# stardist/stardist

Measured on AMD Instinct MI355X. Metric: predict_instances() Mpix/s (2D) + Mvox/s (3D) end-to-end at 1/2/4/8 GPU, higher is better.
Workload: dtype f32

## Files before the change

stardist_amd/csrc/common.h:

```cpp
#pragma once
#include <hip/hip_runtime.h>
#include <stdint.h>
#include <stdio.h>
#include <string.h>

namespace sd {

char* err_buf();
void set_error(const char* fmt, ...);

#define SD_CHECK(expr)                                                                   \
  do {                                                                                   \
    hipError_t _e = (expr);                                                              \
    if (_e != hipSuccess) {                                                              \
      sd::set_error("%s:%d: %s -> %s", __FILE__, __LINE__, #expr, hipGetErrorString(_e)); \
      return -1;                                                                         \
    }                                                                                    \
  } while (0)

#define SD_LAUNCH_CHECK() SD_CHECK(hipGetLastError())

class Arena {
 public:
  int begin(hipStream_t stream);
  void* take(size_t bytes);
  template <typename T> T* take_n(size_t n) { return (T*)take((n ? n : 1) * sizeof(T)); }
  void release();
  size_t capacity() const;
 private:
  enum { kMaxChunks = 64 };
  void* base_[kMaxChunks] = {};
  size_t cap_[kMaxChunks] = {};
  int n_ = 0, cur_ = 0;
  size_t off_ = 0;
};
Arena& arena();

hipStream_t side_stream();

enum { kMaxDevices = 64 };
int resident_grid(const void* kernel, int threads, int* cache);

int cu_count();
int allow_dynamic_lds(const void* const* kernels, int n, int bytes, bool* done);

static inline int div_up(long long a, long long b) { return (int)((a + b - 1) / b); }

enum Option { OPT_NMS3D_VOLUME_BOUNDS, OPT_NMS3D_CONE_MAP, OPT_NMS3D_REFINE_MESH, OPT_PROBE_TIER, OPT_PROBE_NO_GENERAL, OPT_TRACE, OPT_NMS3D_TAIL_BATCH, OPT_NMS3D_SPLIT_EXACT, OPT_CONV_F16_WGS, OPT_NMS2D_PAIR_LANES, OPT_NMS2D_AREA_BOUNDS, OPT_NMS2D_DEFER_UNDECIDED, OPT_NMS2D_STRICT, OPT_NMS2D_NBR_SINGLE, OPT_NMS3D_NBR_SINGLE, OPT_NMS2D_DEFER_MAX, OPT_NMS3D_BOUNDS_REUSE, OPT_NMS3D_DEFER_EXACT, OPT_NMS3D_BOUNDS_LEAN, OPT_COUNT };
int option(Option o);

#ifdef SD_DEBUG_SWITCHES
int tuning_env(const char* name, int dflt);
#else
static inline int tuning_env(const char*, int dflt) { return dflt; }
#endif

}
```

stardist_amd/csrc/lib.hip:

```cpp
#include "common.h"
#include "../../include/stardist_hip.h"
#include <stdarg.h>
#include <stdlib.h>
#include <mutex>

namespace sd {

static thread_local char g_err[1024] = "";
char* err_buf() { return g_err; }
void set_error(const char* fmt, ...) {
  va_list ap;
  va_start(ap, fmt);
  vsnprintf(g_err, sizeof(g_err), fmt, ap);
  va_end(ap);
}

static int g_opt[OPT_COUNT] = {1, 1, 2, 1, 0, 0, 1, 3, 2, 64, 1, 2, 0, 1, 1, 16384, 1, 3, 1};
static const char* const g_opt_name[OPT_COUNT] = {"nms3d_volume_bounds", "nms3d_cone_map", "nms3d_refine_mesh", "probe_tier", "probe_no_general", "trace", "nms3d_tail_batch", "nms3d_split_exact", "conv_f16_workgroups_per_cu", "nms2d_pair_lanes", "nms2d_area_bounds", "nms2d_defer_undecided", "nms2d_strict", "nms2d_neighbours_single_pass", "nms3d_neighbours_single_pass", "nms2d_defer_max", "nms3d_bounds_reuse", "nms3d_defer_exact", "nms3d_bounds_lean"};
int option(Option o) { return g_opt[o]; }
#ifdef SD_DEBUG_SWITCHES
int tuning_env(const char* name, int dflt) { const char* e = getenv(name); return e ? atoi(e) : dflt; }
#endif

static Arena g_arena[kMaxDevices];
Arena& arena() {
  int d = 0;
  if (hipGetDevice(&d) != hipSuccess || d < 0 || d >= kMaxDevices) d = 0;
  return g_arena[d];
}

hipStream_t side_stream() {
  static std::mutex mu;
  static hipStream_t st[kMaxDevices] = {};
  int d = 0;
  if (hipGetDevice(&d) != hipSuccess || d < 0 || d >= kMaxDevices) { set_error("side_stream: no current device"); return nullptr; }
  std::lock_guard<std::mutex> lock(mu);
  if (!st[d] && hipStreamCreateWithFlags(&st[d], hipStreamNonBlocking) != hipSuccess) { st[d] = nullptr; set_error("side_stream: cannot create a stream"); }
  return st[d];
}

int resident_grid(const void* kernel, int threads, int* cache) {
  static std::mutex mu;
  int d = 0;
  if (hipGetDevice(&d) != hipSuccess || d < 0 || d >= kMaxDevices) { set_error("resident_grid: no current device"); return 0; }
  std::lock_guard<std::mutex> lock(mu);
  if (!cache[d]) {
    int per_cu = 0, cus = 0;
    if (hipOccupancyMaxActiveBlocksPerMultiprocessor(&per_cu, kernel, threads, 0) != hipSuccess ||
        hipDeviceGetAttribute(&cus, hipDeviceAttributeMultiprocessorCount, d) != hipSuccess || per_cu <= 0 || cus <= 0) {
      set_error("resident_grid: occupancy query failed");
      return 0;
    }
    cache[d] = per_cu * cus;
  }
  return cache[d];
}

int cu_count() {
  static std::mutex mu;
  static int n_cu[kMaxDevices] = {};
  int d = 0;
// ... 82 lines not shown
```

stardist_amd/csrc/nms2d.hip:

```cpp
#include <type_traits>

#include "common.h"
#include "clip_sweep.h"
#include "clip_beam.h"
#include "area_bounds.h"
#include "poly_pass.h"
#include "nms_rounds.h"
#include "../../include/stardist_hip.h"
#include <hipcub/hipcub.hpp>
#include <math.h>
#include <stdlib.h>
#include <vector>

namespace {

using sdclip::i64;

__device__ __forceinline__ float wave_min(float v) { for (int o = 32; o; o >>= 1) v = fminf(v, __shfl_xor(v, o)); return v; }
__device__ __forceinline__ float wave_max(float v) { for (int o = 32; o; o >>= 1) v = fmaxf(v, __shfl_xor(v, o)); return v; }
__device__ __forceinline__ i64 wave_sum(i64 v) { for (int o = 32; o; o >>= 1) v += __shfl_xor(v, o); return v; }

__global__ void __launch_bounds__(256) k_build(const float* __restrict__ dist, const float* __restrict__ pts,
                                               const float2* __restrict__ sincos, int N, int R,
                                               int* __restrict__ vx, int* __restrict__ vy, int4* __restrict__ bbox,
// ... 654 lines not shown
                                                             const unsigned char* __restrict__ decided, const unsigned char* __restrict__ state) {
  const unsigned long long n = *nPtr, first = firstPtr ? *firstPtr : 0u;
  for (unsigned long long t = first + (unsigned long long)blockIdx.x * 256 + threadIdx.x; t < n; t += (unsigned long long)gridDim.x * 256) {
    if (decided && decided[t]) continue;
    const int2 ij = pairs[t];
    if (pair_j_suppressed(state, ij)) continue;
    const unsigned int k = atomicAdd(&cursor[pair_bucket(pts, ij, key)], 1u);
    if (k < cap) order[k] = (unsigned int)t;
  }
}

__global__ void k_count_after(unsigned int* out, const unsigned int* total, const unsigned int* first) { *out = *total > *first ? *total - *first : 0u; }

}

namespace sd {
int clip_full_pairs(const int2* d_pairs, const unsigned int* d_idx, const unsigned int* d_n, unsigned int cap, int R, const int* d_vx, const int* d_vy,
                    const float* d_area, float thr, unsigned char* d_state, unsigned char* d_supp, unsigned int* d_errCount, hipStream_t stream);
}

namespace {
struct Counters { int nU, nK, nS, left; unsigned long long nPairs; unsigned int nSpill, nExact, nErr, nDecided, nSkipped; };

template <int MAXV, int SPREP>
struct BeamPath {
  typedef sdclip::PolyPrep<MAXV> Prep;
  static constexpr size_t prep_stride = sizeof(Prep);
  static constexpr bool two_tiers = MAXV == 32;
  static int prepare(const int* vx, const int* vy, int N, int R, sdarea::PolyProps* props, void* prep, hipStream_t s) {
    if constexpr (MAXV == 32) {
      if (sdpass::launch_poly_pass(vx, vy, N, R, props, prep, s)) { sd::set_error("sd_nms2d: launch of the per-polygon pass failed"); return -1; }
      return 0;
    } else {
      const size_t lds = sdclip::PrepWork<sdclip::LdsStorage<SPREP>, MAXV>::lds_bytes() + 64;
      hipLaunchKernelGGL((k_prepare<MAXV, SPREP>), dim3(sd::div_up(N, SPREP)), dim3(SPREP), lds, s, vx, vy, N, R, (Prep*)prep);
      SD_LAUNCH_CHECK();
      return 0;
    }
  }
  static int tier1(const int2* pairs, const unsigned int* idx, const unsigned long long* nPairs, const unsigned int* first, const void* prep, const float* area,
                   float thr, unsigned char* state, unsigned char* supp, PairQueues q, hipStream_t s) {
    const int lanes = sd::option(sd::OPT_NMS2D_PAIR_LANES);
    if (lanes == 32) {
      static const size_t lds32 = beam_lds_bytes<MAXV, 8, 6, 4, 32>();
      hipLaunchKernelGGL((k_pairs_beam<MAXV, 8, 6, 4, 32, unsigned long long>), dim3(256 * 8), dim3(32), lds32, s, pairs, idx, nPairs, first, (const Prep*)prep, area, thr, state, supp, q);
    } else if (lanes == 6464) {
// ... 87 lines not shown
  hipStream_t s = (hipStream_t)stream_;
  if (n_polys <= 0) return 0;
  if (n_rays < 1 || n_rays > 256) { sd::set_error("sd_nms2d_build: n_rays=%d unsupported (1..256)", n_rays); return -1; }
  sd::Arena& A = sd::arena();
  if (A.begin(s)) return -1;
  int* gstats = nullptr;
  if (launch_build(A, s, d_dist, d_points, n_polys, n_rays, d_vx, d_vy, (int4*)d_bbox, d_radius, d_area, &gstats, nullptr)) return -1;
  SD_CHECK(hipMemcpyAsync(d_gstats, gstats, 5 * sizeof(int), hipMemcpyDeviceToDevice, s));
  SD_CHECK(hipStreamSynchronize(s));
  return 0;
}

namespace {
struct SideEvents {
  hipEvent_t props = nullptr, prep = nullptr;
  ~SideEvents() { if (props) (void)hipEventDestroy(props); if (prep) (void)hipEventDestroy(prep); }
  int init() { SD_CHECK(hipEventCreateWithFlags(&props, hipEventDisableTiming)); SD_CHECK(hipEventCreateWithFlags(&prep, hipEventDisableTiming)); return 0; }
};

struct Nms2d {
  hipStream_t s; const float *dist, *pts; int N, R, use_kdtree, use_bbox; float thr; bool wantStats; sd::Arena& A;
  bool areaBounds = false, singlePass = false, ordered = false, decide = false, deferOn = false, trace = false;
  int tailT = -1, deferFrom = 0, keyMode = 2; unsigned int deferMax = 0;
  hipStream_t side = nullptr; sd::SideJoin sideJoin; SideEvents sideEv;
  Timer broadTimer, pairTimer, fullTimer, replayTimer;
  double ns_pairs = 0, ns_full = 0, ns_pre = 0; long long n_pair_launches = 0;
  int *vx = nullptr, *vy = nullptr, *candCell = nullptr, *gstats = nullptr; int4* bbox = nullptr; float *radius = nullptr, *area = nullptr;
  unsigned char* state = nullptr; void* prep = nullptr; size_t prepStride = 0; sdarea::PolyProps* props = nullptr;
  GridP g; NmsFlags f; float max_dist = 0, reach = 0;
  int by_bbox = 0, *cellStart = nullptr, *nbrCount = nullptr, *nbrLow = nullptr, *Ucur = nullptr; i64* nbrStart = nullptr; CellRec* cellRec = nullptr;
  void* scanTmp = nullptr; size_t scanBytes = 0; Deferred dfr{nullptr, nullptr, nullptr, nullptr, nullptr, 0};
  NbrLists L{}; i64 totalNbr = 0;
  unsigned long long pairCap = 0, *nOrdered = nullptr; int2* pairs = nullptr; unsigned char *decided = nullptr, *defKind = nullptr;
  unsigned int qCap = 0, *spillPairs = nullptr, *exactPairs = nullptr, *pairOrder = nullptr, *bucketHist = nullptr, *firstNew = nullptr, *nNewExact = nullptr, *nJoinDef = nullptr;
  int *Unext = nullptr, *K = nullptr, *Sl = nullptr, decideGrid = 0; Counters *d_cnt = nullptr, h;
  int nU = 0, rounds = 0; bool forceTail = false;
  i64 nDeferred = 0, nUndecDeferredUpper = 0, totalPairs = 0, totalExact = 0, totalSpill = 0, totalUndecDeferred = 0, totalDecided = 0, totalSkipped = 0;
  unsigned char* supp = nullptr; unsigned int* segStart = nullptr; int* segCnt = nullptr;

  Nms2d(hipStream_t s_, const float* dist_, const float* pts_, int N_, int R_, int use_kdtree_, int use_bbox_, float thr_, bool wantStats_)
      : s(s_), dist(dist_), pts(pts_), N(N_), R(R_), use_kdtree(use_kdtree_), use_bbox(use_bbox_), thr(thr_), wantStats(wantStats_), A(sd::arena()) {}

  int plan() {
    if (R < 1 || R > 256) { sd::set_error("sd_nms2d: n_rays=%d unsupported (1..256)", R); return -1; }
    if (A.begin(s)) return -1;
    if (wantStats && (broadTimer.init() || pairTimer.init() || fullTimer.init())) return -1;
    trace = wantStats && sd::option(sd::OPT_TRACE) != 0;
    areaBounds = R <= 32 && R >= 3 && sd::option(sd::OPT_NMS2D_AREA_BOUNDS) != 0 && sd::option(sd::OPT_NMS2D_STRICT) == 0;
    singlePass = sd::option(sd::OPT_NMS2D_NBR_SINGLE) != 0;
    static const bool pairSort = sd::tuning_env("SD_NMS_PAIR_SORT", 1) != 0;
    static const int pairKey = sd::tuning_env("SD_NMS_PAIR_KEY", 2);
    ordered = pairSort && R <= 32;
    keyMode = pairKey;
    decide = areaBounds && ordered;
    static const int tailDiv = sd::tuning_env("SD_NMS_TAIL_DIV", 6);
    static const int tailMax = sd::tuning_env("SD_NMS_TAIL_MAX", 65536);
    tailT = tailDiv > 0 ? ((N / tailDiv) < tailMax ? (N / tailDiv) : tailMax) : -1;
    static const bool deferEnv = sd::tuning_env("SD_NMS_DEFER", 1) != 0;
    deferOn = tailT >= 0 && deferEnv;
    deferFrom = (deferOn && decide) ? sd::option(sd::OPT_NMS2D_DEFER_UNDECIDED) : 0;
    deferMax = (unsigned int)(sd::option(sd::OPT_NMS2D_DEFER_MAX) > 0 ? sd::option(sd::OPT_NMS2D_DEFER_MAX) : 0);
    side = sd::side_stream();
    if (!side || sideEv.init()) return -1;
    return 0;
  }

  int build() {
    vx = A.take_n<int>((size_t)N * R);
    vy = A.take_n<int>((size_t)N * R);
    bbox = A.take_n<int4>(N);
    radius = A.take_n<float>(N);
    area = A.take_n<float>(N);
    state = A.take_n<unsigned char>(N);
    candCell = A.take_n<int>(N);
    prepStride = prep_stride(R);
    prep = A.take((size_t)N * prepStride);
    if (areaBounds) props = (sdarea::PolyProps*)A.take((size_t)N * sizeof(sdarea::PolyProps));
    if (!vx || !vy || !bbox || !radius || !area || !state || !candCell || !prep || (areaBounds && !props)) return -1;
    return launch_build(A, s, dist, pts, N, R, vx, vy, bbox, radius, area, &gstats, broadTimer.a);
  }

  int fork_side() {
    if (sideJoin.begin(s, side) || prepare_polys(vx, vy, N, R, props, prep, side)) return -1;
    SD_CHECK(hipEventRecord(sideEv.props, side));
    SD_CHECK(hipEventRecord(sideEv.prep, side));
    return 0;
  }

  int build_grid() {
    int gs[8];
    SD_CHECK(hipMemcpyAsync(gs, gstats, sizeof(gs), hipMemcpyDeviceToHost, s));
    SD_CHECK(hipStreamSynchronize(s));
    memcpy(&max_dist, &gs[0], 4);
    reach = (max_dist + 1.f) * 1.0001f + 1e-3f;
    by_bbox = (thr >= 0.f || use_bbox) ? 1 : 0;
    float cs = 0.5f * reach;
    if (!(cs >= 1.f)) cs = 1.f;
    for (;;) {
      g.ny = (int)(((double)gs[2] - gs[1]) / cs) + 1;
      g.nx = (int)(((double)gs[4] - gs[3]) / cs) + 1;
      if ((long long)g.ny * g.nx <= (1ll << 26)) break;
      cs *= 2.f;
    }
    g.y0 = (float)gs[1]; g.x0 = (float)gs[3]; g.inv_cs = 1.f / cs;
    const int nCells = g.ny * g.nx;
    int* cellCount = A.take_n<int>(2 * ((size_t)nCells + 1));
    int* cellFill = cellCount ? cellCount + nCells + 1 : nullptr;
    cellStart = A.take_n<int>(nCells + 1);
    cellRec = (CellRec*)A.take((size_t)N * sizeof(CellRec));
    nbrCount = A.take_n<int>(N + 1);
    nbrStart = A.take_n<i64>(N + 1);
    nbrLow = A.take_n<int>(N + 1);
    if (!cellCount || !cellStart || !cellRec || !nbrCount || !nbrStart || !nbrLow) return -1;
    SD_CHECK(hipMemsetAsync(cellCount, 0, 2 * ((size_t)nCells + 1) * sizeof(int), s));
    hipLaunchKernelGGL(k_cell_count, dim3(sd::div_up(N, 256)), dim3(256), 0, s, pts, N, g, cellCount, candCell);
// ... 9 lines not shown
                       (singlePass || wantStats) ? nbrCount : (int*)nullptr);
    SD_LAUNCH_CHECK();
    Ucur = A.take_n<int>(N);
    dfr.pend = A.take_n<unsigned char>(N);
    dfr.head = A.take_n<int>(N);
    dfr.count = A.take_n<unsigned int>(1);
    if (!Ucur || !dfr.pend || !dfr.head || !dfr.count) return -1;
    hipLaunchKernelGGL(k_round_lists_init, dim3(sd::div_up(N, 256)), dim3(256), 0, s, N, Ucur, state, dfr.pend, dfr.head, dfr.count);
    f.use_kdtree = use_kdtree; f.use_bbox = use_bbox; f.thr_nonneg = (thr >= 0.f); f.thr = thr; f.max_dist = max_dist;
    return 0;
  }

  int build_lists() {
    const int nbBlocks = (sd::div_up(N, 4) + 7) & ~7;
    L.count = nbrCount; L.low = nbrLow; L.start = nbrStart; L.lowOnly = true; L.wantSlotTotal = wantStats;
    auto launch_neighbours = [&](int mode, const NbrLists& l) {
      auto go = [&](auto kern, const i64* start, int* nbr, int* waitOn) {
        hipLaunchKernelGGL(kern, dim3(nbBlocks), dim3(256), 0, s, N, g, f, cellRec, cellStart, nbrCount, nbrLow, start, nbr, waitOn, by_bbox, reach);
      };
      if (mode == 0) go(k_neighbours<0>, nullptr, nullptr, nullptr);
      else if (mode == 1) go(k_neighbours<1>, nbrStart, l.nbr, l.waitOn);
      else go(k_neighbours<2>, nbrStart, l.nbr, l.waitOn);
    };
    const int rc = build_neighbour_lists(A, s, N, singlePass, scanTmp, scanBytes, launch_neighbours, [&]() { return fork_side(); }, L);
    if (rc > 0)
      sd::set_error("sd_nms2d: %lld neighbour entries for %d candidates exceed the capacity of one call (2^31 - 1): shard the input "
                    "(predict_instances_sharded / predict_instances_big)", (long long)L.total, N);
    if (rc) return -1;
    totalNbr = 2 * L.total;
    SD_CHECK(hipStreamWaitEvent(s, sideEv.props, 0));
    float ms = 0;
    if (broadTimer.stop(s) || broadTimer.wait() || broadTimer.ms(&ms)) return -1;
    ns_pre = ms * 1e6;
    return 0;
  }

  int begin_rounds() {
    pairCap = (unsigned long long)(totalNbr / 2 + 64);
    qCap = (unsigned int)(pairCap < (1ull << 30) ? pairCap : (1ull << 30));
    Unext = A.take_n<int>(N);
    K = A.take_n<int>(N);
    pairs = A.take_n<int2>(pairCap);
    spillPairs = A.take_n<unsigned int>(qCap);
    exactPairs = A.take_n<unsigned int>(qCap);
    Sl = A.take_n<int>(N);
    d_cnt = (Counters*)A.take(sizeof(Counters));
    if (ordered) pairOrder = A.take_n<unsigned int>(qCap);
    bucketHist = A.take_n<unsigned int>(2 * PAIR_BUCKETS);
    nOrdered = A.take_n<unsigned long long>(1);
    if (decide) decided = A.take_n<unsigned char>(pairCap);
    firstNew = A.take_n<unsigned int>(1);
    nNewExact = A.take_n<unsigned int>(1);
    if (!Unext || !K || !pairs || !spillPairs || !exactPairs || !Sl || !d_cnt || !bucketHist || !nOrdered || !firstNew || !nNewExact || (ordered && !pairOrder) ||
        (decide && !decided)) return -1;
    static int decideGridOf[sd::kMaxDevices] = {};
    decideGrid = decide ? sd::resident_grid((const void*)k_pairs_decide, 256, decideGridOf) : 0;
    if (decide && decideGrid <= 0) return -1;
    dfr.cap = qCap;
    if (deferOn) {
      dfr.pairs = A.take_n<int2>(qCap);
      dfr.next = A.take_n<int>(qCap);
      if (!dfr.pairs || !dfr.next) return -1;
    }
    if (deferFrom > 0) {
      defKind = A.take_n<unsigned char>(qCap); nJoinDef = A.take_n<unsigned int>(1);
      if (!defKind || !nJoinDef) return -1;
      SD_CHECK(hipMemsetAsync(defKind, 0, qCap, s));
    }
    nU = N;
    return 0;
  }

  int order_pairs(unsigned char* suppOut, const unsigned int* first) {
    static const int modes[6][3] = {{1, 32, 32}, {1, 64, 16}, {1, 64, 64}, {16, 16, 16}, {16, 32, 8}, {4, 32, 32}};
    const int* md = modes[keyMode >= 0 && keyMode < 6 ? keyMode : 2];
    const PairKey key{(const char*)prep, prepStride, 1.f / (4.f * (max_dist + 1.f)), md[0], md[1], md[2]};
    SD_CHECK(hipMemsetAsync(bucketHist, 0, PAIR_BUCKETS * sizeof(unsigned int), s));
    if (decided)
      hipLaunchKernelGGL(k_pairs_decide, dim3(decideGrid), dim3(256), 0, s, pairs, &d_cnt->nPairs, first, vx, vy, R, props, area, thr, state, suppOut,
                         decided, &d_cnt->nDecided);
    if (!suppOut && deferFrom > 0 && rounds >= deferFrom)
      hipLaunchKernelGGL(k_defer_undecided, dim3(256), dim3(256), 0, s, pairs, &d_cnt->nPairs, &d_cnt->nDecided, deferMax, decided, state, dfr, defKind, &d_cnt->nErr);
    const unsigned int* bfirst = (suppOut && deferFrom > 0) ? nullptr : first;
    SD_CHECK(hipStreamWaitEvent(s, sideEv.prep, 0));
    const unsigned char* liveState = suppOut ? nullptr : state;
    hipLaunchKernelGGL(k_pair_bucket_count, dim3(512), dim3(256), 0, s, pairs, &d_cnt->nPairs, bfirst, pts, key, bucketHist, decided, liveState,
                       &d_cnt->nSkipped);
    hipLaunchKernelGGL(k_pair_bucket_scan, dim3(1), dim3(1024), 0, s, bucketHist, bucketHist + PAIR_BUCKETS, nOrdered);
    hipLaunchKernelGGL(k_pair_bucket_scatter, dim3(512), dim3(256), 0, s, pairs, &d_cnt->nPairs, bfirst, pts, key, bucketHist + PAIR_BUCKETS,
                       pairOrder, qCap, decided, liveState);
    SD_LAUNCH_CHECK();
    return 0;
  }

  int sweep_pairs(unsigned char* suppOut) {
    const unsigned int* first = suppOut ? firstNew : nullptr;
    if (pairTimer.start(s)) return -1;
    if (!ordered) SD_CHECK(hipStreamWaitEvent(s, sideEv.prep, 0));
    else if (order_pairs(suppOut, first)) return -1;
    const Sweep w{s, R, vx, vy, prep, area, thr, pairs, spillPairs, exactPairs, qCap, d_cnt, state, suppOut};
// ... 11 lines not shown
      return fullTimer.stop(s);
    };
    if (ordered) return sweep_tiers(w, pairOrder, nOrdered, nullptr, pairTimer, general);
    return sweep_tiers(w, nullptr, &d_cnt->nPairs, first, pairTimer, general);
  }

  int account(const char* what) {
    if (check_sweep("sd_nms2d", h, qCap, h.nPairs > pairCap,
                    " or the deferred-pair list (with more than 64 rays: at least that many; the launch stops at the first)")) return -1;
    totalPairs += (i64)h.nPairs; totalExact += h.nExact; totalSpill += h.nSpill; totalDecided += h.nDecided; totalSkipped += h.nSkipped;
    if (wantStats) {
      float ms = 0, ms2 = 0;
      if (pairTimer.ms(&ms) || fullTimer.ms(&ms2)) return -1;
      if (h.nPairs) { ns_pairs += ms * 1e6; ++n_pair_launches; }
      ns_full += ms2 * 1e6;
      if (trace) printf("%s %d: nU=%d nK=%d pairs=%llu decided by the area enclosure=%u j already suppressed=%u spill=%u exact=%u pair_kernel=%.3f ms general_path=%.3f ms\n", what, rounds, h.nU, h.nK, h.nPairs, h.nDecided, h.nSkipped, h.nSpill, h.nExact, ms, ms2);
    }
    return 0;
  }

  int run_round() {
    ++rounds;
    if (tailT >= 0 && ((nU <= tailT && rounds > 1) || forceTail)) return tail_batch();
    SD_CHECK(hipMemsetAsync(d_cnt, 0, sizeof(Counters), s));
    hipLaunchKernelGGL(k_round_triage, dim3(sd::div_up(nU, 1024)), dim3(1024), 0, s, Ucur, nU, state, L.waitOn, Unext, K, Sl, (int*)d_cnt, dfr.pend);
    const int wgrid = sd::div_up(nU, 4) < 2048 ? sd::div_up(nU, 4) : 2048;
    hipLaunchKernelGGL(k_round_scan, dim3(wgrid), dim3(256), 0, s, Sl, state, nbrStart, nbrLow, L.nbr, L.waitOn, Unext, K, (int*)d_cnt, dfr.pend);
    hipLaunchKernelGGL(k_round_emit, dim3(wgrid), dim3(256), 0, s, K, &d_cnt->nK, state, g, cellRec, cellStart, by_bbox, reach, f, pts, bbox,
                       radius, area, pairs, &d_cnt->nPairs, pairCap);
    SD_LAUNCH_CHECK();
    if (sweep_pairs(nullptr)) return -1;
    SD_CHECK(hipMemcpyAsync(&h, d_cnt, sizeof(Counters), hipMemcpyDeviceToHost, s));
    SD_CHECK(hipStreamSynchronize(s));
    if (h.nK == 0 && h.nU > 0) {
      if (deferOn && (nDeferred > 0 || nUndecDeferredUpper > 0) && !forceTail) forceTail = true;
      else { sd::set_error("sd_nms2d: greedy scan made no progress (internal error)"); return -1; }
    }
    if (deferOn) nDeferred += h.nExact;
    if (deferFrom > 0 && rounds >= deferFrom && h.nPairs > h.nDecided && h.nPairs - h.nDecided <= deferMax) nUndecDeferredUpper += (i64)(h.nPairs - h.nDecided);
    if (account("round")) return -1;
    nU = h.nU;
    int* t = Ucur; Ucur = Unext; Unext = t;
    return 0;
  }

  int tail_batch() {
    if (!supp) { supp = A.take_n<unsigned char>(pairCap); segStart = A.take_n<unsigned int>(N); segCnt = A.take_n<int>(N); }
    if (!supp || !segStart || !segCnt) return -1;
    SD_CHECK(hipMemsetAsync(d_cnt, 0, sizeof(Counters), s));
    SD_CHECK(hipMemsetAsync(supp, 0, pairCap, s));
    if (deferFrom > 0) {
      hipLaunchKernelGGL(k_tail_init2, dim3(64), dim3(256), 0, s, dfr, defKind, pairs, exactPairs, &d_cnt->nPairs, &d_cnt->nExact, firstNew, decided, state,
                         &d_cnt->nSkipped);
      hipLaunchKernelGGL(k_copy_u32, dim3(1), dim3(1), 0, s, nJoinDef, &d_cnt->nExact);
    } else
      hipLaunchKernelGGL(k_tail_init, dim3(64), dim3(256), 0, s, dfr, pairs, exactPairs, &d_cnt->nPairs, &d_cnt->nExact, firstNew);
    if (deferOn && nDeferred > 0 && nDeferred < (i64)qCap) {
      if (sideJoin.begin(s, side)) return -1;
      if (sd::clip_full_pairs(pairs, exactPairs, deferFrom > 0 ? nJoinDef : firstNew, qCap, R, vx, vy, area, thr, state, supp, &d_cnt->nErr, side)) return -1;
      if (sideJoin.end(side)) return -1;
    }
    const int wg = sd::div_up(nU, 4) < 2048 ? sd::div_up(nU, 4) : 2048;
    hipLaunchKernelGGL(k_tail_emit, dim3(wg), dim3(256), 0, s, Ucur, nU, state, nbrStart, nbrLow, L.nbr, f, pts, bbox, radius, area, pairs,
                       &d_cnt->nPairs, pairCap, segStart, segCnt);
    SD_LAUNCH_CHECK();
    if (sweep_pairs(supp)) return -1;
    if (trace && (replayTimer.init() || replayTimer.start(s))) return -1;
    for (int it = 0; it < 10; ++it)
      hipLaunchKernelGGL(k_tail_step, dim3(sd::div_up(nU, 256)), dim3(256), 0, s, Ucur, nU, state, pairs, supp, segStart, segCnt, pairCap, dfr.head, dfr.next);
    hipLaunchKernelGGL(k_tail_resolve, dim3(1), dim3(1024), 0, s, Ucur, nU, state, pairs, supp, segStart, segCnt, pairCap, &d_cnt->left, dfr.head, dfr.next);
    SD_LAUNCH_CHECK();
    if (trace) {
      float ms = 0;
      if (replayTimer.stop(s) || replayTimer.wait() || replayTimer.ms(&ms)) return -1;
      printf("tail replay (10 steps + resolve loop): %.3f ms\n", ms);
    }
    unsigned int hDefTotal = (unsigned int)nDeferred;
    SD_CHECK(hipMemcpyAsync(&h, d_cnt, sizeof(Counters), hipMemcpyDeviceToHost, s));
    if (deferFrom > 0) SD_CHECK(hipMemcpyAsync(&hDefTotal, dfr.count, sizeof(unsigned int), hipMemcpyDeviceToHost, s));
    SD_CHECK(hipStreamSynchronize(s));
    h.nU = nU; h.nK = 0;
    if (deferFrom > 0) totalUndecDeferred = (i64)hDefTotal - nDeferred;
    const unsigned long long counted = deferFrom > 0 ? (unsigned long long)hDefTotal : (unsigned long long)nDeferred;
    if (counted <= h.nPairs) h.nPairs -= counted;
    if ((i64)h.nExact >= nDeferred) h.nExact -= (unsigned int)nDeferred;
    if (account("tail batch after round")) return -1;
    if (h.left) { sd::set_error("sd_nms2d: tail batch left candidates undecided (internal error)"); return -1; }
    nU = 0;
    return 0;
  }

  int report(uint8_t* d_keep, int64_t* stats, int verbose) {
    hipLaunchKernelGGL(k_keep, dim3(sd::div_up(N, 256)), dim3(256), 0, s, state, d_keep, N);
    SD_LAUNCH_CHECK();
    SD_CHECK(hipStreamSynchronize(s));
    if (stats) { stats[0] = totalPairs; stats[1] = totalExact; stats[2] = rounds; stats[3] = totalNbr;
                 stats[4] = (int64_t)ns_pairs; stats[5] = n_pair_launches; stats[6] = (int64_t)ns_full; stats[7] = (int64_t)ns_pre;
                 stats[8] = totalSpill; stats[9] = totalDecided; stats[10] = totalUndecDeferred; stats[11] = totalSkipped;
                 stats[12] = L.slotTotal; stats[13] = L.slots ? 1 : 0; }
    if (verbose) {
      printf("NMS: %lld pair intersections (%lld on the exact-join path), %d greedy rounds, %lld neighbour entries\n",
             (long long)totalPairs, (long long)totalExact, rounds, (long long)totalNbr);
      fflush(stdout);
    }
    return 0;
  }
};
}

extern "C" int sd_nms2d_device(const float* d_dist, const float* d_points, int n_polys, int n_rays, int use_kdtree,
                               int use_bbox, int verbose, float threshold, uint8_t* d_keep, int64_t* stats,
                               void* stream_) {
  hipStream_t s = (hipStream_t)stream_;
  if (stats) memset(stats, 0, 16 * sizeof(int64_t));
  if (n_polys <= 0) return 0;
  Nms2d c(s, d_dist, d_points, n_polys, n_rays, use_kdtree, use_bbox, threshold, stats != nullptr);
  if (c.plan()) return -1;
  if (verbose) {
// ... 221 lines not shown
```

stardist_amd/csrc/nms3d.hip:

```cpp
#include <algorithm>

#include "common.h"
#include "geom3d.h"
#include "nms_rounds.h"
#include "nms3d_shared.h"
#include "nms3d_lds.h"
#include "nms3d_hiv.h"
#include "nms3d_mesh.h"
#include "nms3d_hull.h"
#include "../../include/stardist_hip.h"
#include <hipcub/hipcub.hpp>
#include <math.h>
#include <vector>

namespace {

typedef long long i64;

__device__ __forceinline__ const float* stage_rows(const float* __restrict__ dist, int N, int R, float* lds, int staged) {
  if (!staged) return dist + (size_t)min((int)(blockIdx.x * blockDim.x + threadIdx.x), N - 1) * R;
  const int i0 = blockIdx.x * blockDim.x;
  const int rows = min((int)blockDim.x, N - i0);
  const float* src = dist + (size_t)i0 * R;
  const int pitch = sdl::RowsLds{R}.pitch();
// ... 1217 lines not shown
      }
      SD_LAUNCH_CHECK();
      SD_CHECK(hipMemcpyAsync(&left, d_left, sizeof(int), hipMemcpyDeviceToHost, s));
      SD_CHECK(hipStreamSynchronize(s));
      if (++sweeps > N / 8 + 4) { sd::set_error("sd_nms3d: tail replay does not converge (internal error)"); return -1; }
    }
    return 0;
  }

  int run_round() {
    ++rounds;
    const bool tail = rounds > 1 && (nU <= tailT || forceTail);
    SD_CHECK(hipMemsetAsync(d_cnt, 0, sizeof(Counters), s));
    if (tail) {
      if (!supEdges) {
        supEdges = A.take_n<int2>(pairCap); supCount = A.take_n<unsigned int>(1); blocked = A.take_n<unsigned char>(N); d_left = A.take_n<int>(1);
        if (!supEdges || !supCount || !blocked || !d_left) return -1;
      }
      SD_CHECK(hipMemsetAsync(supCount, 0, sizeof(unsigned int), s));
      SD_CHECK(hipMemsetAsync(blocked, 0, N, s));
      if (hDef) hipLaunchKernelGGL(k_seed3, dim3(sd::div_up(hDef, 256)), dim3(256), 0, s, dfr, dfrCount, dfrCap, pairs3, &d_cnt->nP3);
      h.nK = nU; h.nU = 0;
    } else {
      hipLaunchKernelGGL(k_round_triage, dim3(sd::div_up(nU, 256)), dim3(256), 0, s, Ucur, nU, state, L.waitOn, Unext, Kl, Sl, (int*)d_cnt, (const unsigned char*)pend);
      const int wgrid = sd::div_up(nU, 4) < 2048 ? sd::div_up(nU, 4) : 2048;
      hipLaunchKernelGGL(k_round_scan, dim3(wgrid), dim3(256), 0, s, Sl, state, nbrStart, nbrLow, L.nbr, L.waitOn, Unext, Kl, (int*)d_cnt, (const unsigned char*)pend);
      SD_LAUNCH_CHECK();
    }
    const SuppSink sink = tail ? SuppSink{state, supEdges, supCount, pairCap} : SuppSink{state, nullptr, nullptr, 0u};
    {
      const int egrid = sd::div_up(nU, 4) < 2048 ? sd::div_up(nU, 4) : 2048;
      hipLaunchKernelGGL(k_round_emit3, dim3(egrid), dim3(256), 0, s, tail ? Ucur : Kl, tail ? nU : 0, tail ? (const int*)nullptr : (const int*)&d_cnt->nK, sink, tail ? 1 : 0,
                         nbrStart, nbrCount, (const int*)L.nbr, f, an, pts, bbox, volume, r_outer, r_outer_iso, r_inner_iso, pairs3, &d_cnt->nP3, pairCap, d_st);
      SD_LAUNCH_CHECK();
      SD_CHECK(hipMemcpyAsync(&h, d_cnt, sizeof(Counters), hipMemcpyDeviceToHost, s));
      SD_CHECK(hipStreamSynchronize(s));
    }
    if (!tail && h.nK == 0 && h.nU > 0) {
      if (!hDef) { sd::set_error("sd_nms3d: greedy scan made no progress (internal error)"); return -1; }
      forceTail = true;
      nU = h.nU;
      std::swap(Ucur, Unext);
      return 0;
    }
    const int nUndecided = tail ? 0 : h.nU;
    if (h.nP3 > pairCap) { sd::set_error("sd_nms3d: pair queue overflow (internal error)"); return -1; }
    if (h.nP3 > 0) {
// ... 108 lines not shown
```

stardist_amd/csrc/nms_rounds.h:

```cpp
#pragma once
#include "common.h"
#include <hipcub/hipcub.hpp>

namespace sd {
struct SideJoin {
  hipEvent_t fork = nullptr, done = nullptr;
  bool pending = false;
  ~SideJoin() { if (pending) (void)hipEventSynchronize(done); if (fork) (void)hipEventDestroy(fork); if (done) (void)hipEventDestroy(done); }
  int begin(hipStream_t s, hipStream_t side) {
    if (!fork) { SD_CHECK(hipEventCreateWithFlags(&fork, hipEventDisableTiming)); SD_CHECK(hipEventCreateWithFlags(&done, hipEventDisableTiming)); }
    SD_CHECK(hipEventRecord(fork, s));
    SD_CHECK(hipStreamWaitEvent(side, fork, 0));
    return 0;
  }
  int end(hipStream_t side) { SD_CHECK(hipEventRecord(done, side)); pending = true; return 0; }
  int join(hipStream_t s) { if (pending) { SD_CHECK(hipStreamWaitEvent(s, done, 0)); pending = false; } return 0; }
};
}

namespace {

struct Timer {
  hipEvent_t a = nullptr, b = nullptr;
  ~Timer() { if (a) (void)hipEventDestroy(a); if (b) (void)hipEventDestroy(b); }
  int init() { SD_CHECK(hipEventCreate(&a)); SD_CHECK(hipEventCreate(&b)); return 0; }
  int start(hipStream_t s) { if (a) SD_CHECK(hipEventRecord(a, s)); return 0; }
  int stop(hipStream_t s) { if (a) SD_CHECK(hipEventRecord(b, s)); return 0; }
  int wait() { if (a) SD_CHECK(hipEventSynchronize(b)); return 0; }
  int ms(float* out) { *out = 0; if (a) SD_CHECK(hipEventElapsedTime(out, a, b)); return 0; }
};

enum { ST_UNDECIDED = 0, ST_KEPT = 1, ST_SUPPRESSED = 2 };

#define WAIT_NONE (-2)
#define WAIT_SCAN (-1)

struct NmsFlags { int use_kdtree, use_bbox, thr_nonneg; float thr, max_dist; };

__global__ void k_iota(int* a, int n) { int i = blockIdx.x * blockDim.x + threadIdx.x; if (i < n) a[i] = i; }
__global__ void k_keep(const unsigned char* __restrict__ state, unsigned char* __restrict__ keep, int n) {
  int i = blockIdx.x * blockDim.x + threadIdx.x;
  if (i < n) keep[i] = (state[i] != ST_SUPPRESSED);
}

__global__ void __launch_bounds__(256) k_sum_halves(const int* __restrict__ nLow, const int* __restrict__ nHigh, int N, unsigned long long* total) {
  __shared__ unsigned long long ws[4];
  unsigned long long v = 0;
  for (int i = blockIdx.x * 256 + threadIdx.x; i < N; i += gridDim.x * 256) v += (unsigned long long)(nLow[i] + (nHigh ? nHigh[i] : 0));
  for (int o = 32; o; o >>= 1) v += __shfl_xor(v, o);
  if ((threadIdx.x & 63) == 0) ws[threadIdx.x >> 6] = v;
  __syncthreads();
  if (threadIdx.x == 0) atomicAdd(total, ws[0] + ws[1] + ws[2] + ws[3]);
}

__global__ void __launch_bounds__(1024) k_round_triage(const int* __restrict__ U, int nU, const unsigned char* __restrict__ state,
                                                       const int* __restrict__ waitOn, int* __restrict__ Unext, int* __restrict__ K,
                                                       int* __restrict__ S, int* counters ,
                                                       const unsigned char* __restrict__ pend) {
  const int t = blockIdx.x * blockDim.x + threadIdx.x;
  const int lane = threadIdx.x & 63, wave = threadIdx.x >> 6, nw = blockDim.x >> 6;
  int kind = 0, i = -1;
  if (t < nU) {
    i = U[t];
    if (state[i] != ST_SUPPRESSED) {
      const int wo = waitOn[i];
      if (pend && pend[i]) kind = 1;
      else if (wo == WAIT_NONE) kind = 2;
      else if (wo >= 0 && state[wo] == ST_UNDECIDED) kind = 1;
      else kind = 3;
    }
  }
  __shared__ int wcnt[3][16];
  __shared__ int bbase[3];
#pragma unroll
  for (int q = 1; q <= 3; ++q) {
    const unsigned long long m = __ballot(kind == q);
    if (lane == 0) wcnt[q - 1][wave] = __popcll(m);
  }
  __syncthreads();
  if (threadIdx.x < 3) {
    int sum = 0;
// ... 56 lines not shown
    }
    if (nbuf > 60) flush();
  }
  flush();
}

struct NbrLists {
  int* count; int* low; long long* start;
  int* nbr; int* waitOn;
  long long total, slotTotal;
  bool slots;
  bool lowOnly;
  bool wantSlotTotal;
};

struct WidenCount { __host__ __device__ __forceinline__ long long operator()(const int& v) const { return (long long)v; } };
inline hipError_t exclusive_sum_i64(void* tmp, size_t& tmpBytes, const int* count, long long* start, int n, hipStream_t s) {
  hipcub::TransformInputIterator<long long, WidenCount, const int*> in(count, WidenCount());
  return hipcub::DeviceScan::ExclusiveScan(tmp, tmpBytes, in, start, hipcub::Sum(), (long long)0, n, s);
}

template <class LaunchNeighbours, class BeforeLists>
int build_neighbour_lists(sd::Arena& A, hipStream_t s, int N, bool singlePass, void* scanTmp, size_t scanBytes,
                          LaunchNeighbours launch, BeforeLists beforeLists, NbrLists& L) {
  L.nbr = nullptr; L.waitOn = nullptr; L.total = 0; L.slotTotal = 0; L.slots = false;
  if (singlePass || L.wantSlotTotal) {
    SD_CHECK(exclusive_sum_i64(scanTmp, scanBytes, L.count, L.start, N + 1, s));
    SD_CHECK(hipMemcpyAsync(&L.slotTotal, L.start + N, sizeof(long long), hipMemcpyDeviceToHost, s));
    SD_CHECK(hipStreamSynchronize(s));
    L.slots = singlePass && L.slotTotal >= 0 && L.slotTotal < 0x7fffffffll;
  }
  if (L.slots) {
    L.nbr = A.take_n<int>((size_t)L.slotTotal);
    if (!L.nbr) L.slots = false;
  }
  if (L.slots && beforeLists()) return -1;
  if (!L.slots) {
    SD_CHECK(hipMemsetAsync(L.count, 0, (N + 1) * sizeof(int), s));
    launch(0, L);
    SD_LAUNCH_CHECK();
    SD_CHECK(exclusive_sum_i64(scanTmp, scanBytes, L.count, L.start, N + 1, s));
    SD_CHECK(hipMemcpyAsync(&L.total, L.start + N, sizeof(long long), hipMemcpyDeviceToHost, s));
    SD_CHECK(hipStreamSynchronize(s));
    if (beforeLists()) return -1;
  }
  if (L.total < 0 || L.total >= 0x7fffffffll) return 1;
  if (!L.slots) L.nbr = A.take_n<int>((size_t)L.total);
  L.waitOn = A.take_n<int>(N);
  if (!L.nbr || !L.waitOn) return -1;
  if (L.slots) {
    unsigned long long* d_total = A.take_n<unsigned long long>(1);
    if (!d_total) return -1;
    SD_CHECK(hipMemsetAsync(d_total, 0, sizeof(unsigned long long), s));
    launch(2, L);
    hipLaunchKernelGGL(k_sum_halves, dim3(sd::div_up(N, 256) < 1024 ? sd::div_up(N, 256) : 1024), dim3(256), 0, s, L.low, L.lowOnly ? (const int*)nullptr : L.count, N, d_total);
    SD_LAUNCH_CHECK();
    unsigned long long tot = 0;
    SD_CHECK(hipMemcpyAsync(&tot, d_total, sizeof(tot), hipMemcpyDeviceToHost, s));
    SD_CHECK(hipStreamSynchronize(s));
    L.total = (long long)tot;
  } else {
    launch(1, L);
    SD_LAUNCH_CHECK();
  }
  return 0;
}

}
```

Measured before the change: 341.3.

## Speculatively queue next NMS round and read counters via mapped host memory

Replaces the small device-to-host memcpy plus stream synchronize readbacks in 2D NMS with a one-thread kernel that writes into mapped pinned host memory, followed by an event wait. The round loop now double-buffers the counters and enqueues the next round's triage/scan/emit before the host reads the current counters, with the triage kernel clamping its length to a device-computed live count. It also defers the join on the side-stream properties event and the broad-phase timer read until later. The aim is to hide per-round host round-trip latency. In exchange the code gets more complex, and a speculatively queued round is wasted when the host decides to stop or switch to the tail path.

```diff
diff --git a/stardist_amd/csrc/common.h b/stardist_amd/csrc/common.h
--- a/stardist_amd/csrc/common.h
+++ b/stardist_amd/csrc/common.h
@@ -38,6 +38,9 @@
 
 hipStream_t side_stream();
 
+struct HostWords { void* host; void* dev; size_t bytes; };
+HostWords host_words();
+
 enum { kMaxDevices = 64 };
 int resident_grid(const void* kernel, int threads, int* cache);
 
diff --git a/stardist_amd/csrc/lib.hip b/stardist_amd/csrc/lib.hip
--- a/stardist_amd/csrc/lib.hip
+++ b/stardist_amd/csrc/lib.hip
@@ -37,6 +37,29 @@
   std::lock_guard<std::mutex> lock(mu);
   if (!st[d] && hipStreamCreateWithFlags(&st[d], hipStreamNonBlocking) != hipSuccess) { st[d] = nullptr; set_error("side_stream: cannot create a stream"); }
   return st[d];
+}
+
+HostWords host_words() {
+  static std::mutex mu;
+  static HostWords hw[kMaxDevices] = {};
+  static bool asked[kMaxDevices] = {};
+  const HostWords none{nullptr, nullptr, 0};
+  int d = 0;
+  if (hipGetDevice(&d) != hipSuccess || d < 0 || d >= kMaxDevices) return none;
+  std::lock_guard<std::mutex> lock(mu);
+  if (!asked[d]) {
+    asked[d] = true;
+    const size_t bytes = 4096;
+    void *h = nullptr, *dv = nullptr;
+    int canMap = 0;
+    if (hipDeviceGetAttribute(&canMap, hipDeviceAttributeCanMapHostMemory, d) == hipSuccess && canMap &&
+        hipHostMalloc(&h, bytes, hipHostMallocMapped) == hipSuccess) {
+      if (hipHostGetDevicePointer(&dv, h, 0) == hipSuccess && dv) { memset(h, 0, bytes); hw[d] = HostWords{h, dv, bytes}; }
+      else (void)hipHostFree(h);
+    }
+    (void)hipGetLastError();
+  }
+  return hw[d];
 }
 
 int resident_grid(const void* kernel, int threads, int* cache) {
diff --git a/stardist_amd/csrc/nms2d.hip b/stardist_amd/csrc/nms2d.hip
--- a/stardist_amd/csrc/nms2d.hip
+++ b/stardist_amd/csrc/nms2d.hip
@@ -700,6 +700,24 @@
 namespace {
 struct Counters { int nU, nK, nS, left; unsigned long long nPairs; unsigned int nSpill, nExact, nErr, nDecided, nSkipped; };
 
+struct RoundRule { int tailT; unsigned long long pairCap; unsigned int qCap; };
+__host__ __device__ inline bool sweep_overflowed(const Counters& c, const RoundRule& r) { return c.nPairs > r.pairCap || c.nSpill > r.qCap || c.nExact > r.qCap; }
+__host__ __device__ inline bool plain_round_follows(const Counters& c, const RoundRule& r) {
+  if (sweep_overflowed(c, r) || c.nErr) return false;
+  if (c.nU <= 0 || c.nK == 0) return false;
+  return !(r.tailT >= 0 && c.nU <= r.tailT);
+}
+__global__ void k_round_publish(const Counters* __restrict__ cnt, unsigned int* __restrict__ mapped, RoundRule rule, int* __restrict__ nextLen) {
+  if (blockIdx.x || threadIdx.x) return;
+  const Counters c = *cnt;
+  *nextLen = plain_round_follows(c, rule) ? c.nU : 0;
+  if (mapped) {
+    const unsigned int* w = (const unsigned int*)cnt;
+    for (int i = 0; i < (int)(sizeof(Counters) / 4); ++i) mapped[i] = w[i];
+    __threadfence_system();
+  }
+}
+
 template <int MAXV, int SPREP>
 struct BeamPath {
   typedef sdclip::PolyPrep<MAXV> Prep;
@@ -833,7 +851,8 @@
   hipStream_t s; const float *dist, *pts; int N, R, use_kdtree, use_bbox; float thr; bool wantStats; sd::Arena& A;
   bool areaBounds = false, singlePass = false, ordered = false, decide = false, deferOn = false, trace = false;
   int tailT = -1, deferFrom = 0, keyMode = 2; unsigned int deferMax = 0;
-  hipStream_t side = nullptr; sd::SideJoin sideJoin; SideEvents sideEv;
+  hipStream_t side = nullptr; sd::SideJoin sideJoin; SideEvents sideEv; bool forked = false, propsJoined = false;
+  Readback rb;
   Timer broadTimer, pairTimer, fullTimer, replayTimer;
   double ns_pairs = 0, ns_full = 0, ns_pre = 0; long long n_pair_launches = 0;
   int *vx = nullptr, *vy = nullptr, *candCell = nullptr, *gstats = nullptr; int4* bbox = nullptr; float *radius = nullptr, *area = nullptr;
@@ -845,12 +864,14 @@
   unsigned long long pairCap = 0, *nOrdered = nullptr; int2* pairs = nullptr; unsigned char *decided = nullptr, *defKind = nullptr;
   unsigned int qCap = 0, *spillPairs = nullptr, *exactPairs = nullptr, *pairOrder = nullptr, *bucketHist = nullptr, *firstNew = nullptr, *nNewExact = nullptr, *nJoinDef = nullptr;
   int *Unext = nullptr, *K = nullptr, *Sl = nullptr, decideGrid = 0; Counters *d_cnt = nullptr, h;
+  Counters* cntBlk[2] = {nullptr, nullptr}; int cb = 0, *nextLen = nullptr; bool headQueued = false;
   int nU = 0, rounds = 0; bool forceTail = false;
   i64 nDeferred = 0, nUndecDeferredUpper = 0, totalPairs = 0, totalExact = 0, totalSpill = 0, totalUndecDeferred = 0, totalDecided = 0, totalSkipped = 0;
   unsigned char* supp = nullptr; unsigned int* segStart = nullptr; int* segCnt = nullptr;
 
   Nms2d(hipStream_t s_, const float* dist_, const float* pts_, int N_, int R_, int use_kdtree_, int use_bbox_, float thr_, bool wantStats_)
       : s(s_), dist(dist_), pts(pts_), N(N_), R(R_), use_kdtree(use_kdtree_), use_bbox(use_bbox_), thr(thr_), wantStats(wantStats_), A(sd::arena()) {}
+  ~Nms2d() { if (forked) (void)hipEventSynchronize(sideEv.prep); }
 
   int plan() {
     if (R < 1 || R > 256) { sd::set_error("sd_nms2d: n_rays=%d unsupported (1..256)", R); return -1; }
@@ -872,7 +893,7 @@
     deferFrom = (deferOn && decide) ? sd::option(sd::OPT_NMS2D_DEFER_UNDECIDED) : 0;
     deferMax = (unsigned int)(sd::option(sd::OPT_NMS2D_DEFER_MAX) > 0 ? sd::option(sd::OPT_NMS2D_DEFER_MAX) : 0);
     side = sd::side_stream();
-    if (!side || sideEv.init()) return -1;
+    if (!side || sideEv.init() || rb.init()) return -1;
     return 0;
   }
 
@@ -895,13 +916,15 @@
     if (sideJoin.begin(s, side) || prepare_polys(vx, vy, N, R, props, prep, side)) return -1;
     SD_CHECK(hipEventRecord(sideEv.props, side));
     SD_CHECK(hipEventRecord(sideEv.prep, side));
+    forked = true;
+    static const bool serialPass = sd::tuning_env("SD_NMS_SERIAL_PASS", 0) != 0;
+    if (serialPass) SD_CHECK(hipStreamWaitEvent(s, sideEv.prep, 0));
     return 0;
   }
 
   int build_grid() {
     int gs[8];
-    SD_CHECK(hipMemcpyAsync(gs, gstats, sizeof(gs), hipMemcpyDeviceToHost, s));
-    SD_CHECK(hipStreamSynchronize(s));
+    if (rb.fetch(s, gstats, RB_GSTATS, gs, sizeof(gs))) return -1;
     memcpy(&max_dist, &gs[0], 4);
     reach = (max_dist + 1.f) * 1.0001f + 1e-3f;
     by_bbox = (thr >= 0.f || use_bbox) ? 1 : 0;
@@ -957,17 +980,13 @@
       else if (mode == 1) go(k_neighbours<1>, nbrStart, l.nbr, l.waitOn);
       else go(k_neighbours<2>, nbrStart, l.nbr, l.waitOn);
     };
-    const int rc = build_neighbour_lists(A, s, N, singlePass, scanTmp, scanBytes, launch_neighbours, [&]() { return fork_side(); }, L);
+    const int rc = build_neighbour_lists(A, s, N, singlePass, scanTmp, scanBytes, launch_neighbours, [&]() { return fork_side(); }, L, &rb);
     if (rc > 0)
       sd::set_error("sd_nms2d: %lld neighbour entries for %d candidates exceed the capacity of one call (2^31 - 1): shard the input "
                     "(predict_instances_sharded / predict_instances_big)", (long long)L.total, N);
     if (rc) return -1;
     totalNbr = 2 * L.total;
-    SD_CHECK(hipStreamWaitEvent(s, sideEv.props, 0));
-    float ms = 0;
-    if (broadTimer.stop(s) || broadTimer.wait() || broadTimer.ms(&ms)) return -1;
-    ns_pre = ms * 1e6;
-    return 0;
+    return broadTimer.stop(s);
   }
 
   int begin_rounds() {
@@ -979,14 +998,16 @@
     spillPairs = A.take_n<unsigned int>(qCap);
     exactPairs = A.take_n<unsigned int>(qCap);
     Sl = A.take_n<int>(N);
-    d_cnt = (Counters*)A.take(sizeof(Counters));
+    cntBlk[0] = (Counters*)A.take(sizeof(Counters)); cntBlk[1] = (Counters*)A.take(sizeof(Counters));
+    d_cnt = cntBlk[cb = 0];
+    nextLen = A.take_n<int>(1);
     if (ordered) pairOrder = A.take_n<unsigned int>(qCap);
     bucketHist = A.take_n<unsigned int>(2 * PAIR_BUCKETS);
     nOrdered = A.take_n<unsigned long long>(1);
     if (decide) decided = A.take_n<unsigned char>(pairCap);
     firstNew = A.take_n<unsigned int>(1);
     nNewExact = A.take_n<unsigned int>(1);
-    if (!Unext || !K || !pairs || !spillPairs || !exactPairs || !Sl || !d_cnt || !bucketHist || !nOrdered || !firstNew || !nNewExact || (ordered && !pairOrder) ||
+    if (!Unext || !K || !pairs || !spillPairs || !exactPairs || !Sl || !cntBlk[0] || !cntBlk[1] || !nextLen || !bucketHist || !nOrdered || !firstNew || !nNewExact || (ordered && !pairOrder) ||
         (decide && !decided)) return -1;
     static int decideGridOf[sd::kMaxDevices] = {};
     decideGrid = decide ? sd::resident_grid((const void*)k_pairs_decide, 256, decideGridOf) : 0;
@@ -1011,6 +1032,7 @@
     const int* md = modes[keyMode >= 0 && keyMode < 6 ? keyMode : 2];
     const PairKey key{(const char*)prep, prepStride, 1.f / (4.f * (max_dist + 1.f)), md[0], md[1], md[2]};
     SD_CHECK(hipMemsetAsync(bucketHist, 0, PAIR_BUCKETS * sizeof(unsigned int), s));
+    if (decided && !propsJoined) { SD_CHECK(hipStreamWaitEvent(s, sideEv.props, 0)); propsJoined = true; }
     if (decided)
       hipLaunchKernelGGL(k_pairs_decide, dim3(decideGrid), dim3(256), 0, s, pairs, &d_cnt->nPairs, first, vx, vy, R, props, area, thr, state, suppOut,
                          decided, &d_cnt->nDecided);
@@ -1068,25 +1090,40 @@
   int run_round() {
     ++rounds;
     if (tailT >= 0 && ((nU <= tailT && rounds > 1) || forceTail)) return tail_batch();
+    if (!headQueued && round_head(nullptr)) return -1;
+    headQueued = false;
+    if (sweep_pairs(nullptr)) return -1;
+    const RoundRule rule{tailT, pairCap, qCap};
+    hipLaunchKernelGGL(k_round_publish, dim3(1), dim3(64), 0, s, d_cnt, (unsigned int*)(rb.host ? rb.dev + RB_COUNTERS + 64 * cb : nullptr), rule, nextLen);
+    SD_LAUNCH_CHECK();
+    if (!rb.host) SD_CHECK(hipMemcpyAsync(&h, d_cnt, sizeof(Counters), hipMemcpyDeviceToHost, s));
+    if (rb.mark(s)) return -1;
+    const int cbRead = cb;
+    { int* t = Ucur; Ucur = Unext; Unext = t; }
+    d_cnt = cntBlk[cb ^= 1];
+    if (round_head(nextLen)) return -1;
+    if (rb.wait()) return -1;
+    rb.read(RB_COUNTERS + 64 * cbRead, &h, sizeof(Counters));
+    if (h.nK == 0 && h.nU > 0) {
+      if (deferOn && (nDeferred > 0 || nUndecDeferredUpper > 0) && !forceTail) forceTail = true;
+      else { sd::set_error("sd_nms2d: greedy scan made no progress (internal error)"); return -1; }
+    }
+    if (deferOn) nDeferred += h.nExact;
+    if (deferFrom > 0 && rounds >= deferFrom && h.nPairs > h.nDecided && h.nPairs - h.nDecided <= deferMax) nUndecDeferredUpper += (i64)(h.nPairs - h.nDecided);
+    if (account("round")) return -1;
+    nU = h.nU;
+    headQueued = plain_round_follows(h, rule);
+    return 0;
+  }
+
+  int round_head(const int* live) {
     SD_CHECK(hipMemsetAsync(d_cnt, 0, sizeof(Counters), s));
-    hipLaunchKernelGGL(k_round_triage, dim3(sd::div_up(nU, 1024)), dim3(1024), 0, s, Ucur, nU, state, L.waitOn, Unext, K, Sl, (int*)d_cnt, dfr.pend);
+    hipLaunchKernelGGL(k_round_triage, dim3(sd::div_up(nU, 1024)), dim3(1024), 0, s, Ucur, nU, state, L.waitOn, Unext, K, Sl, (int*)d_cnt, dfr.pend, live);
     const int wgrid = sd::div_up(nU, 4) < 2048 ? sd::div_up(nU, 4) : 2048;
     hipLaunchKernelGGL(k_round_scan, dim3(wgrid), dim3(256), 0, s, Sl, state, nbrStart, nbrLow, L.nbr, L.waitOn, Unext, K, (int*)d_cnt, dfr.pend);
     hipLaunchKernelGGL(k_round_emit, dim3(wgrid), dim3(256), 0, s, K, &d_cnt->nK, state, g, cellRec, cellStart, by_bbox, reach, f, pts, bbox,
                        radius, area, pairs, &d_cnt->nPairs, pairCap);
     SD_LAUNCH_CHECK();
-    if (sweep_pairs(nullptr)) return -1;
-    SD_CHECK(hipMemcpyAsync(&h, d_cnt, sizeof(Counters), hipMemcpyDeviceToHost, s));
-    SD_CHECK(hipStreamSynchronize(s));
-    if (h.nK == 0 && h.nU > 0) {
-      if (deferOn && (nDeferred > 0 || nUndecDeferredUpper > 0) && !forceTail) forceTail = true;
-      else { sd::set_error("sd_nms2d: greedy scan made no progress (internal error)"); return -1; }
-    }
-    if (deferOn) nDeferred += h.nExact;
-    if (deferFrom > 0 && rounds >= deferFrom && h.nPairs > h.nDecided && h.nPairs - h.nDecided <= deferMax) nUndecDeferredUpper += (i64)(h.nPairs - h.nDecided);
-    if (account("round")) return -1;
-    nU = h.nU;
-    int* t = Ucur; Ucur = Unext; Unext = t;
     return 0;
   }
 
@@ -1122,9 +1159,11 @@
       printf("tail replay (10 steps + resolve loop): %.3f ms\n", ms);
     }
     unsigned int hDefTotal = (unsigned int)nDeferred;
-    SD_CHECK(hipMemcpyAsync(&h, d_cnt, sizeof(Counters), hipMemcpyDeviceToHost, s));
-    if (deferFrom > 0) SD_CHECK(hipMemcpyAsync(&hDefTotal, dfr.count, sizeof(unsigned int), hipMemcpyDeviceToHost, s));
-    SD_CHECK(hipStreamSynchronize(s));
+    if (rb.publish(s, d_cnt, RB_COUNTERS, &h, sizeof(Counters))) return -1;
+    if (deferFrom > 0 && rb.publish(s, dfr.count, RB_DEF_COUNT, &hDefTotal, sizeof(unsigned int))) return -1;
+    if (rb.mark(s) || rb.wait()) return -1;
+    rb.read(RB_COUNTERS, &h, sizeof(Counters));
+    if (deferFrom > 0) rb.read(RB_DEF_COUNT, &hDefTotal, sizeof(unsigned int));
     h.nU = nU; h.nK = 0;
     if (deferFrom > 0) totalUndecDeferred = (i64)hDefTotal - nDeferred;
     const unsigned long long counted = deferFrom > 0 ? (unsigned long long)hDefTotal : (unsigned long long)nDeferred;
@@ -1140,6 +1179,7 @@
     hipLaunchKernelGGL(k_keep, dim3(sd::div_up(N, 256)), dim3(256), 0, s, state, d_keep, N);
     SD_LAUNCH_CHECK();
     SD_CHECK(hipStreamSynchronize(s));
+    if (wantStats) { float ms = 0; if (broadTimer.ms(&ms)) return -1; ns_pre = ms * 1e6; }
     if (stats) { stats[0] = totalPairs; stats[1] = totalExact; stats[2] = rounds; stats[3] = totalNbr;
                  stats[4] = (int64_t)ns_pairs; stats[5] = n_pair_launches; stats[6] = (int64_t)ns_full; stats[7] = (int64_t)ns_pre;
                  stats[8] = totalSpill; stats[9] = totalDecided; stats[10] = totalUndecDeferred; stats[11] = totalSkipped;
diff --git a/stardist_amd/csrc/nms3d.hip b/stardist_amd/csrc/nms3d.hip
--- a/stardist_amd/csrc/nms3d.hip
+++ b/stardist_amd/csrc/nms3d.hip
@@ -1263,7 +1263,7 @@
       if (hDef) hipLaunchKernelGGL(k_seed3, dim3(sd::div_up(hDef, 256)), dim3(256), 0, s, dfr, dfrCount, dfrCap, pairs3, &d_cnt->nP3);
       h.nK = nU; h.nU = 0;
     } else {
-      hipLaunchKernelGGL(k_round_triage, dim3(sd::div_up(nU, 256)), dim3(256), 0, s, Ucur, nU, state, L.waitOn, Unext, Kl, Sl, (int*)d_cnt, (const unsigned char*)pend);
+      hipLaunchKernelGGL(k_round_triage, dim3(sd::div_up(nU, 256)), dim3(256), 0, s, Ucur, nU, state, L.waitOn, Unext, Kl, Sl, (int*)d_cnt, (const unsigned char*)pend, (const int*)nullptr);
       const int wgrid = sd::div_up(nU, 4) < 2048 ? sd::div_up(nU, 4) : 2048;
       hipLaunchKernelGGL(k_round_scan, dim3(wgrid), dim3(256), 0, s, Sl, state, nbrStart, nbrLow, L.nbr, L.waitOn, Unext, Kl, (int*)d_cnt, (const unsigned char*)pend);
       SD_LAUNCH_CHECK();
diff --git a/stardist_amd/csrc/nms_rounds.h b/stardist_amd/csrc/nms_rounds.h
--- a/stardist_amd/csrc/nms_rounds.h
+++ b/stardist_amd/csrc/nms_rounds.h
@@ -30,6 +30,37 @@
   int ms(float* out) { *out = 0; if (a) SD_CHECK(hipEventElapsedTime(out, a, b)); return 0; }
 };
 
+enum { RB_GSTATS = 0, RB_SLOT_TOTAL = 32, RB_LIST_TOTAL = 40, RB_DEF_COUNT = 48, RB_COUNTERS = 64  };
+__global__ void k_publish(const unsigned int* __restrict__ src, unsigned int* __restrict__ dst, int n) {
+  if (blockIdx.x == 0 && threadIdx.x == 0) {
+    for (int i = 0; i < n; ++i) dst[i] = src[i];
+    __threadfence_system();
+  }
+}
+struct Readback {
+  char *host = nullptr, *dev = nullptr; hipEvent_t ev = nullptr;
+  ~Readback() { if (ev) (void)hipEventDestroy(ev); }
+  int init() {
+    const sd::HostWords w = sd::host_words();
+    host = (char*)w.host; dev = (char*)w.dev;
+    SD_CHECK(hipEventCreateWithFlags(&ev, hipEventDisableTiming));
+    return 0;
+  }
+  int publish(hipStream_t s, const void* d_src, size_t off, void* dst, size_t bytes) {
+    if (host) { hipLaunchKernelGGL(k_publish, dim3(1), dim3(64), 0, s, (const unsigned int*)d_src, (unsigned int*)(dev + off), (int)(bytes >> 2)); SD_LAUNCH_CHECK(); }
+    else SD_CHECK(hipMemcpyAsync(dst, d_src, bytes, hipMemcpyDeviceToHost, s));
+    return 0;
+  }
+  int mark(hipStream_t s) { SD_CHECK(hipEventRecord(ev, s)); return 0; }
+  int wait() { SD_CHECK(hipEventSynchronize(ev)); return 0; }
+  void read(size_t off, void* dst, size_t bytes) const { if (host) memcpy(dst, host + off, bytes); }
+  int fetch(hipStream_t s, const void* d_src, size_t off, void* dst, size_t bytes) {
+    if (publish(s, d_src, off, dst, bytes) || mark(s) || wait()) return -1;
+    read(off, dst, bytes);
+    return 0;
+  }
+};
+
 enum { ST_UNDECIDED = 0, ST_KEPT = 1, ST_SUPPRESSED = 2 };
 
 #define WAIT_NONE (-2)
@@ -56,7 +87,8 @@
 __global__ void __launch_bounds__(1024) k_round_triage(const int* __restrict__ U, int nU, const unsigned char* __restrict__ state,
                                                        const int* __restrict__ waitOn, int* __restrict__ Unext, int* __restrict__ K,
                                                        int* __restrict__ S, int* counters ,
-                                                       const unsigned char* __restrict__ pend) {
+                                                       const unsigned char* __restrict__ pend, const int* __restrict__ nULive) {
+  if (nULive) { const int live = *nULive; nU = live < nU ? live : nU; }
   const int t = blockIdx.x * blockDim.x + threadIdx.x;
   const int lane = threadIdx.x & 63, wave = threadIdx.x >> 6, nw = blockDim.x >> 6;
   int kind = 0, i = -1;
@@ -159,12 +191,17 @@
 
 template <class LaunchNeighbours, class BeforeLists>
 int build_neighbour_lists(sd::Arena& A, hipStream_t s, int N, bool singlePass, void* scanTmp, size_t scanBytes,
-                          LaunchNeighbours launch, BeforeLists beforeLists, NbrLists& L) {
+                          LaunchNeighbours launch, BeforeLists beforeLists, NbrLists& L, Readback* rb = nullptr) {
+  auto total_of = [&](const void* d_src, size_t off, void* dst) -> int {
+    if (rb) return rb->fetch(s, d_src, off, dst, 8);
+    SD_CHECK(hipMemcpyAsync(dst, d_src, 8, hipMemcpyDeviceToHost, s));
+    SD_CHECK(hipStreamSynchronize(s));
+    return 0;
+  };
   L.nbr = nullptr; L.waitOn = nullptr; L.total = 0; L.slotTotal = 0; L.slots = false;
   if (singlePass || L.wantSlotTotal) {
     SD_CHECK(exclusive_sum_i64(scanTmp, scanBytes, L.count, L.start, N + 1, s));
-    SD_CHECK(hipMemcpyAsync(&L.slotTotal, L.start + N, sizeof(long long), hipMemcpyDeviceToHost, s));
-    SD_CHECK(hipStreamSynchronize(s));
+    if (total_of(L.start + N, RB_SLOT_TOTAL, &L.slotTotal)) return -1;
     L.slots = singlePass && L.slotTotal >= 0 && L.slotTotal < 0x7fffffffll;
   }
   if (L.slots) {
@@ -177,8 +214,7 @@
     launch(0, L);
     SD_LAUNCH_CHECK();
     SD_CHECK(exclusive_sum_i64(scanTmp, scanBytes, L.count, L.start, N + 1, s));
-    SD_CHECK(hipMemcpyAsync(&L.total, L.start + N, sizeof(long long), hipMemcpyDeviceToHost, s));
-    SD_CHECK(hipStreamSynchronize(s));
+    if (total_of(L.start + N, RB_LIST_TOTAL, &L.total)) return -1;
     if (beforeLists()) return -1;
   }
   if (L.total < 0 || L.total >= 0x7fffffffll) return 1;
@@ -193,8 +229,7 @@
     hipLaunchKernelGGL(k_sum_halves, dim3(sd::div_up(N, 256) < 1024 ? sd::div_up(N, 256) : 1024), dim3(256), 0, s, L.low, L.lowOnly ? (const int*)nullptr : L.count, N, d_total);
     SD_LAUNCH_CHECK();
     unsigned long long tot = 0;
-    SD_CHECK(hipMemcpyAsync(&tot, d_total, sizeof(tot), hipMemcpyDeviceToHost, s));
-    SD_CHECK(hipStreamSynchronize(s));
+    if (total_of(d_total, RB_LIST_TOTAL, &tot)) return -1;
     L.total = (long long)tot;
   } else {
     launch(1, L);
```

After: 345.3, median of 6. 1.2% higher.
